# ZhonghuaYi/FocusFlow_official

Measured on AMD Instinct MI355X. Metric: frame-pairs/sec FF-RAFT 384x512 iters=12, higher is better.
Workload: dtype f32 via fp16x3 split operands on the f16 MFMA pipe (f32 accumulate, fp32-level accuracy); 1 GPU; FF-RAFT forward (test_mode), 8 pairs/GPU 384x512, iters=12, fp32 correlation pyramid, random-init weights, ORB-like masks (BASELINE configs[1]); pairs_per_gpu=8, corr_pyramid=fp32, conv_precision=f16x3, hipgraph=False, skip_unused_upsample=False, parallelism=dp1 (independent shards, no collective)

## Files before the change

focusflow_official_amd/_hip.py:

```python
import ctypes as C
import os

_PKG = os.path.dirname(os.path.abspath(__file__))
LIB_PATH = os.path.join(_PKG, "lib", "libfocusflow_hip.so")
if os.environ.get("FF_LAB_LIB"):
    LIB_PATH = os.path.join(_PKG, "lib", os.environ["FF_LAB_LIB"])

ACT_NONE, ACT_RELU, ACT_SIGMOID, ACT_TANH, ACT_LEAKY = 0, 1, 2, 3, 4
W_F32, W_F16X3, W_F16 = 0, 1, 2
MAX_SEG = 3
_fp = C.c_void_p
_ll = C.c_longlong


class FFFusionPair(C.Structure):
    _fields_ = [
        ("x", _fp * 2), ("x_ld", C.c_int * 2), ("xres", _fp * 2), ("xres_ld", C.c_int * 2), ("scale", _fp * 2), ("shift", _fp * 2),
        ("in_act", C.c_int), ("w_frag", _fp * 2), ("bias", _fp * 2), ("w_format", C.c_int), ("y", _fp * 2), ("y_ld", C.c_int * 2),
        ("B", C.c_int), ("HW", C.c_int), ("C", C.c_int),
    ]


class FFEncoderTail(C.Structure):
    _fields_ = [
# ... 83 lines not shown
    "ff_corr_alt_lookup": [_fp, C.POINTER(_fp), C.c_int, _fp, C.c_int, C.c_int, C.c_int, _fp, C.c_int, _fp, _fp],
    "ff_corr_alt_lookup_bwd": [_fp, C.POINTER(_fp), C.POINTER(_fp), C.POINTER(_fp), C.c_int, C.c_int, C.c_int, C.c_int, C.c_int, _fp,
                               C.POINTER(_fp), _fp],
    "ff_act_copy": [_fp, C.c_int, _fp, C.c_int, _ll, C.c_int, C.c_int, _fp],
    "ff_range_probe": [_fp, C.c_int, _ll, C.c_int, _fp, _fp],
    "ff_split_copy": [_fp, C.c_int, _fp, C.c_int, _ll, C.c_int, C.c_int, C.c_int, _fp],
    "ff_coords_init": [_fp, _fp, C.c_int, C.c_int, C.c_int, _fp],
    "ff_forward_interpolate": [_fp, _fp, _fp, C.c_int, C.c_int, C.c_int, _fp],
    "ff_good_features": [_fp, C.c_int, _ll, _ll, _ll, C.c_int, C.c_int, C.c_int, C.c_int, C.c_double, C.c_int, _fp, _fp, _fp, _fp, _fp],
    "ff_frame_ingest": [_fp, _ll, _ll, _ll, _ll, C.c_int, C.c_int, C.c_int, C.c_int, C.c_int, C.c_int, C.c_int, C.c_int, _fp, _fp],
    "ff_pad_replicate": [_fp, C.c_int, _ll, _ll, _ll, C.c_int, C.c_int, C.c_int, C.c_int, C.c_int, C.c_int, C.c_int, _fp, _fp],
    "ff_keypoint_matches": [_fp, _fp, C.c_int, _fp, _ll, _ll, _ll, _ll, C.c_int, C.c_int, C.c_int, C.c_int, C.c_int, C.c_int, C.c_int, _fp, _fp, _fp],
    "ff_tracks_replenish": [_fp, _fp, _fp, _fp, C.c_int, _fp, _fp, C.c_int, C.c_int, C.c_int, C.c_int, C.c_int, _fp, _fp, _fp],
    "ff_tracks_mask": [_fp, _fp, C.c_int, C.c_int, C.c_int, C.c_int, _fp, _fp],
    "ff_tracks_advance": [_fp, _fp, _fp, C.c_int, _fp, _ll, _ll, _ll, _ll, C.c_int, C.c_int, C.c_int, C.c_int, C.c_int, C.c_int, C.c_int, _fp, _fp, _fp,
                          _fp, _fp],
    "ff_fb_dense": [_fp, _ll, _ll, _ll, _ll, _fp, _ll, _ll, _ll, _ll, C.c_int, C.c_int, C.c_int, C.c_int, C.c_int, C.c_int, C.c_int, C.c_float, C.c_float,
                    _fp, _fp, _fp],
    "ff_fb_matches": [_fp, _fp, C.c_int, _fp, _ll, _ll, _ll, _ll, C.c_int, C.c_int, C.c_int, C.c_int, C.c_int, C.c_int, C.c_int, C.c_float, C.c_float,
                      _fp, _fp, _fp, _fp, _fp, _fp],
    "ff_epipolar_ransac": [_fp, _fp, C.c_int, C.c_int, C.c_int, C.c_int, C.c_float, C.c_int, C.c_int, C.c_int, C.c_uint, _fp, C.c_int, _fp, _fp, _fp, _fp,
                           _fp, _fp, _fp, _fp, _fp, _fp, _ll, _fp],
    "ff_epipolar_ransac_hold": [_fp, _fp, C.c_int, C.c_int, C.c_int, C.c_int, C.c_float, C.c_int, C.c_int, C.c_int, C.c_uint, _fp, C.c_int, _fp, _fp, _fp,
                                _fp, _fp, _fp, _fp, _fp, _fp, _fp, _ll, _fp, _fp],
    "ff_homography_ransac": [_fp, _fp, C.c_int, C.c_int, C.c_int, C.c_int, C.c_float, C.c_int, C.c_int, C.c_int, C.c_int, C.c_uint, _fp, C.c_int, _fp, _fp,
                             _fp, _fp, _fp, _fp, _fp, _fp, _fp, _fp, _fp, _ll, _fp],
    "ff_homography_residual": [_fp, _ll, _ll, _ll, _ll, _fp, _fp, C.c_int, C.c_int, C.c_int, _fp, _fp],
    "ff_coords_step": [_fp, _fp, C.c_int, _fp, _fp, C.c_int, C.c_int, C.c_int, C.c_int, _fp],
    "ff_gru_pass": [C.c_int, _fp, C.c_int, _fp, C.c_int, _fp, C.c_int, _fp, C.c_int, _fp, C.c_int, _fp, _fp, _fp, _fp, C.c_int, _fp, C.c_int, _fp, C.c_int,
                    C.c_int, C.c_int, C.c_int, _fp],
    "ff_gru_pass_rec": [C.c_int, _fp, C.c_int, _fp, C.c_int, _fp, C.c_int, _fp, C.c_int, _fp, C.c_int, _fp, _fp, _fp, _fp, C.c_int, _fp, C.c_int, _fp, C.c_int,
                        _fp, _fp, _fp, C.c_int, C.c_int, C.c_int, C.c_int, _fp],
    "ff_fusion_pair_fwd": [C.POINTER(FFFusionPair), _fp],
    "ff_encoder_tail_fwd": [C.POINTER(FFEncoderTail), _fp],
    "ff_conv_s2_pair_fwd": [C.POINTER(FFConvS2Pair), _fp],
    "ff_gru_rh": [_fp, C.c_int, _fp, C.c_int, _fp, C.c_int, _ll, C.c_int, _fp],
    "ff_gru_blend": [_fp, C.c_int, _fp, C.c_int, _fp, C.c_int, _fp, C.c_int, _ll, C.c_int, _fp],
    "ff_upsample_flow": [_fp, C.c_int, _fp, C.c_int, _fp, C.c_int, C.c_int, C.c_int, _fp],
    "ff_nhwc_to_nchw": [_fp, C.c_int, _fp, C.c_int, C.c_int, C.c_int, C.c_int, _fp],
    "ff_conv2d_wgrad": [C.POINTER(FFConvParams), _fp, _ll, _fp, _fp],
    "ff_unpack_conv_wgrad": [_fp, C.c_int, C.c_int, C.c_int, C.c_int, C.c_int, C.c_int, _fp, _fp],
    "ff_pack_conv_weight_dgrad": [_fp, C.c_int, C.c_int, C.c_int, C.c_int, _fp, C.c_int, C.c_int, _fp],
    "ff_act_bwd": [_fp, C.c_int, _fp, C.c_int, _fp, C.c_int, _ll, C.c_int, C.c_int, C.c_int, C.c_float, _fp, _fp],
    "ff_deconv4x4s2_small": [_fp, C.c_int, C.c_int, C.c_int, C.c_int, C.c_int, _fp, _fp, C.c_int, _fp, C.c_int, _fp],
    "ff_dilate2": [_fp, C.c_int, _fp, C.c_int, C.c_int, C.c_int, C.c_int, C.c_int, C.c_int, _fp],
    "ff_norm_bwd": [_fp, C.c_int, _fp, C.c_int, _fp, C.c_int, _fp, _fp, C.c_int, C.c_int, C.c_float, _fp, _fp,
                    C.c_int, _fp, C.c_int, _fp, C.c_int, C.c_int, C.c_int, C.c_int, _fp, _fp],
    "ff_gru_rh_bwd": [_fp, C.c_int, _fp, C.c_int, _fp, C.c_int, _fp, C.c_int, _fp, C.c_int, _ll, C.c_int, _fp],
    "ff_gru_blend_bwd": [_fp, C.c_int, _fp, C.c_int, _fp, C.c_int, _fp, C.c_int, _fp, C.c_int, _fp, C.c_int,
                         _fp, C.c_int, _ll, C.c_int, _fp],
    "ff_upsample_flow_bwd": [_fp, _fp, C.c_int, _fp, C.c_int, _fp, _fp, C.c_int, C.c_int, C.c_int, _fp],
    "ff_upsample_flow_bwd_ex": [_fp, _fp, C.c_int, _fp, C.c_int, _fp, C.c_int, _fp, C.c_float, _fp, C.c_int, C.c_int, C.c_int, _fp],
    "ff_gru_bwd_blend": [_fp, C.c_int, _fp, C.c_int, _fp, C.c_int, _fp, C.c_int, _fp, C.c_int, _fp, C.c_int, _fp, C.c_int, _fp, C.c_int, _fp, C.c_int,
                         _fp, _fp, _ll, C.c_int, _fp],
    "ff_gru_bwd_rh": [_fp, C.c_int, _fp, C.c_int, _fp, C.c_int, _fp, C.c_int, _fp, C.c_int, _fp, C.c_int, C.c_int, _fp, _ll, C.c_int, _fp],
    "ff_gru_bwd_out": [_fp, C.c_int, _fp, C.c_int, _fp, C.c_int, _fp, C.c_int, _fp, C.c_int, _fp, C.c_int, C.c_int, _fp, _ll, C.c_int, _fp],
    "ff_sum_stack": [_fp, C.c_int, _ll, _fp, _fp],
    "ff_pwc_costvolume_fwd": [_fp, C.c_int, _fp, C.c_int, _fp, C.c_int, C.c_int, C.c_int, C.c_int, C.c_int, _fp],
    "ff_pwc_costvolume_fwd_ex": [_fp, C.c_int, _fp, C.c_int, _fp, C.c_int, C.c_int, C.c_int, C.c_int, C.c_int, C.c_int, _fp, C.c_int, _fp],
    "ff_pwc_costvolume_bwd": [_fp, C.c_int, _fp, C.c_int, _fp, C.c_int, C.c_int, C.c_int, C.c_int, C.c_int, _fp],
    "ff_pwc_gout_transpose": [_fp, C.c_int, _fp, C.c_int, C.c_int, C.c_int, C.c_int, _fp],
    "ff_pwc_backwarp": [_fp, C.c_int, _fp, C.c_int, C.c_float, _fp, C.c_int, C.c_int, C.c_int, C.c_int, C.c_int, _fp],
    "ff_loss_prepare": [_fp, _fp, _fp, _fp, C.c_int, C.c_float, _fp, _fp, _fp, C.c_int, C.c_int, C.c_int, _fp],
    "ff_loss_accumulate": [_fp, _fp, _fp, _fp, _fp, C.c_float, C.c_float, C.c_float, _fp, _fp, C.c_int, C.c_int,
                           C.c_int, _fp],
    "ff_epe_metric": [_fp, _fp, _fp, _fp, C.c_int, C.c_int, C.c_int, _fp],
# ... 97 lines not shown
```

focusflow_official_amd/cce.py:

```python
from typing import Tuple, Optional, Sequence

import ctypes
import os
import weakref

import torch
import torch.nn as nn

from . import _hip, fn, ops
from .ops import ACT_NONE, ACT_RELU, ACT_SIGMOID

EPS = 1e-5


_NORM_ON_LOAD = True


_ALL_PACKED = weakref.WeakSet()
_DMA_FRAG = True
_PREPACK = True
_serial = [0]


class PackedConv:
# ... 276 lines not shown
            arr[i] = J
        host = torch.frombuffer(bytearray(bytes(arr)), dtype=torch.uint8)
        cache = owner.__dict__["_ff_pack_table"] = (sig, host.to(device), len(jobs), blk)
    ops.pack_weights_table(cache[1], cache[2], cache[3])
    for (pc, nf, nd, kf, kd), (J, fmt, dfmt) in zip(todo, jobs):
        if nf:
            pc.w, pc.fmt, pc._key = (pc._w_raw if fmt == 0 else pc._w_split), fmt, kf
            pc._gen += 1
        if nd:
            pc.wd, pc.dfmt, pc._dkey = (pc._wd_raw if dfmt == 0 else pc._wd_split), dfmt, kd
    return len(todo)


def train_streams() -> bool:
    v = os.environ.get("FF_TRAIN_STREAMS")
    if v is not None:
        return v != "0"
    return not (torch.distributed.is_available() and torch.distributed.is_initialized())
_BRANCH_STREAMS = True
_branch_streams = {}


def _branch_stream(device):
    key = (torch.device(device).index, torch.cuda.current_stream(device).cuda_stream)
    if key not in _branch_streams:
        _branch_streams[key] = torch.cuda.Stream(device=device)
    return _branch_streams[key]


_FUSION_PAIR = os.environ.get("FF_FUSION_PAIR", "1") != "0"
_PAIR_FUSION = True
_ENCODER_TAIL = True
_S2_PAIR = True
_W_LIMIT = 4094.0


def invalidate_packed(module: nn.Module) -> int:
    ids = {id(p) for p in module.parameters()}
    n = 0
    for pc in list(_ALL_PACKED):
        if id(pc.convs[0]._parameters["weight"]) in ids:
            pc._key = pc._dkey = None
            n += 1
    for m in module.modules():
        if hasattr(m, "_ff_fold"):
            del m._ff_fold
            n += 1
        if getattr(m, "_pair_key", None) is not None:
            m._pair_key = None
            n += 1
        if getattr(m, "_tail_key", None) is not None:
            m._tail_key = None
            n += 1
        if getattr(m, "_mask2_stage_of", None) is not None:
            m._mask2_stage = m._mask2_stage_of = None
            n += 1
    return n


def _make_norm(kind: str, c: int):
    if kind == "batch":
        return nn.BatchNorm2d(c)
    if kind == "instance":
        return nn.InstanceNorm2d(c)
    if kind == "none":
        return nn.Sequential()
# ... 76 lines not shown
            self.mask2img = _FusionConv(2 * c, c)
            self.img2mask = _FusionConv(2 * c, c) if bi_direction else None
        elif fusion_type in ("SA", "CA"):
            unit = _SA if fusion_type == "SA" else _CA
            self.mask2img = unit(c)
            self.img2mask = unit(c) if bi_direction else None
        else:
            raise ValueError(f"Fusion type {fusion_type} not supported.")

    def _paired(self):
        a, b = self.mask2img.conv, self.img2mask.conv
        key = (ops.conv_precision(),) + tuple((t._version, t.data_ptr()) for t in (a.weight, a.bias, b.weight, b.bias))
        if getattr(self, "_pair_key", None) != key:
            c = a.out_channels
            wf = torch.zeros((2 * c, 2 * c, 1, 1), dtype=torch.float32, device=a.weight.device)
            wf[:c, c:] = a.weight.detach()
            wf[c:, :c] = b.weight.detach()
            rows = torch.empty((2 * c, 2 * c), dtype=torch.float32, device=wf.device)
            ops.pack_conv_weight(wf, rows, 2 * c, 0)
            self._pair_w = ops.pack_split(rows)
            self._pair_b = torch.cat([a.bias.detach(), b.bias.detach()]).contiguous()
            self._pair_key = key
        return self._pair_w, self._pair_b

    def _pair_kernel_ok(self, img):
        if not (_FUSION_PAIR and self.fusion_type == "1x1conv" and self.img2mask is not None and not torch.is_grad_enabled()
                and ops.w_format() in (_hip.W_F16X3, _hip.W_F16)):
            return False
        b, h, w, c = img.shape
        tp = ops.fusion_pair_tile(c)
        return tp > 0 and (h * w) % tp == 0

    def run(self, mask, img):
        if self._pair_kernel_ok(img) and mask.shape == img.shape and ops.fusion_pair_inputs_ok(img, mask):
            pa, pb = self.mask2img._p, self.img2mask._p
            (_, ba), (_, bb) = pa.get(), pb.get()
            img_out, mask_out = ops.fusion_pair(img, mask, (pa.frag(), pb.frag()), (ba, bb), ops.w_format())
            return mask_out, img_out
        if isinstance(img, ops.LazyAct):
            img = img.materialise()
        if isinstance(mask, ops.LazyAct):
            mask = mask.materialise()
        if (_PAIR_FUSION and self.fusion_type == "1x1conv" and self.img2mask is not None and not torch.is_grad_enabled()
                and ops.w_format() != 0 and img.shape[3] % 32 == 0 and img.shape == mask.shape):
            c = img.shape[3]
            w, bias = self._paired()
            y = ops.conv2d([img, mask], w, bias, 2 * c, 1, 1, res=img, res2=mask, res_split=c, w_fmt=ops.w_format())
            return y[..., c:], y[..., :c]
        if self.fusion_type in ("SA", "CA"):
            img_out = self.mask2img.run(img, mask)
            mask_out = self.img2mask.run(mask, img) if self.img2mask is not None else mask
        elif self.fusion_type == "concat":
            img_out = fn.conv(self.mask2img._p, [img, mask])
            mask_out = fn.conv(self.img2mask._p, [mask, img]) if self.img2mask is not None else mask
        else:
            img_out = fn.conv(self.mask2img._p, mask, res=img)
            mask_out = fn.conv(self.img2mask._p, img, res=mask) if self.img2mask is not None else mask
        return mask_out, img_out


class _ResidualEncoder(nn.Module):

    def _frame_layers(self, in_channel, output_dim):
        self.norm1 = _make_norm(self.norm_fn, 64)
        self.conv1 = nn.Conv2d(in_channel, 64, 7, stride=2, padding=3)
        self.layer1 = self._stage(64, 64, 1)
        self.layer2 = self._stage(64, 96, 2)
        self.layer3 = self._stage(96, 128, 2)
        self.conv2 = nn.Conv2d(128, output_dim, 1)

    def _init_weights(self):
# ... 188 lines not shown
            return False
        probe = torch.empty((1, h, w, c), device="meta")
        return unit._pair_kernel_ok(probe)

    def _tail_eligible(self) -> bool:
        return (_ENCODER_TAIL and not torch.is_grad_enabled() and ops.w_format() in (_hip.W_F16X3, _hip.W_F16)
                and self.fusion_type in ("1x1conv", "1x1conv-unidirection") and self.fusion5.img2mask is None
                and (self.conv2.in_channels, self.conv2.out_channels) == (128, 256) and self.conv2.weight.is_cuda)

    def _tail_weights(self):
        f4, f5 = self.fusion4, self.fusion5
        convs = [f4.mask2img.conv, self.conv2, self.mask_conv2, f5.mask2img.conv] + ([f4.img2mask.conv] if f4.img2mask is not None else [])
        key = (ops.conv_precision(),) + tuple((t._version, t.data_ptr()) for cv in convs for t in (cv._parameters["weight"], cv._parameters["bias"]))
        if getattr(self, "_tail_key", None) != key:
            if torch.cuda.is_current_stream_capturing():
                return None
            w64 = lambda cv: cv.weight.detach().double().flatten(1)
            b64 = lambda cv: cv.bias.detach().double()
            a4, wx, wm, a5 = (w64(cv) for cv in convs[:4])
            w_x, w_m, bm = wx, wx @ a4 + a5 @ wm, b64(self.mask_conv2)
            if f4.img2mask is not None:
                w_x = wx + a5 @ (wm @ w64(f4.img2mask.conv))
                bm = wm @ b64(f4.img2mask.conv) + bm
            bias = wx @ b64(f4.mask2img.conv) + b64(self.conv2) + a5 @ bm + b64(f5.mask2img.conv)
            wf = torch.cat([w_x, w_m], 1).float()
            self._tail = None
            if float(wf.abs().max()) < _W_LIMIT:
                rows = torch.empty_like(wf)
                ops.pack_conv_weight(wf[:, :, None, None].contiguous(), rows, wf.shape[1], 0)
                self._tail = (ops.pack_frag16(ops.pack_split(rows), wf.shape[0]), bias.float().contiguous())
            self._tail_key = key
        return self._tail

    def forward(self, x, mask):
        b, hh, ww = x.shape[0], x.shape[1], x.shape[2]
        lz1 = self._lazy_for(self.fusion1, 64, hh // 2, ww // 2)
        lz2 = self._lazy_for(self.fusion2, 64, hh // 2, ww // 2)
        lz3 = self._lazy_for(self.fusion3, 96, hh // 4, ww // 4)
        m, x = self._branches(lambda t: self._conv_norm(t, self._mstem, self.mask_norm1, ACT_RELU, lazy=lz1),
                              lambda t: self._run_stem(t, lz1), mask, x)
        m, x = self.fusion1.run(m, x)
        m, x = self._branches(lambda t: self._run_stage(self.mask_layer1, t, lz2), lambda t: self._run_stage(self.layer1, t, lz2), m, x)
        m, x = self.fusion2.run(m, x)
        m, x = self._branches(lambda t: self._run_stage(self.mask_layer2, t, lz3), lambda t: self._run_stage(self.layer2, t, lz3), m, x)
        m, x = self.fusion3.run(m, x)
        tail = self._tail_weights() if self._tail_eligible() else None
        lz4 = tail is not None and self.norm_fn == "instance"
        m, x = self._branches(lambda t: self._run_stage(self.mask_layer3, t, lz4), lambda t: self._run_stage(self.layer3, t, lz4), m, x)
        if tail is not None and ops.encoder_tail_inputs_ok(x, m):
            return ops.encoder_tail(x, m, tail[0], tail[1], ops.w_format())
        m, x = self.fusion4.run(m, x)
        m, x = fn.conv(self._mout, m), self._run_out(x)
        m, x = self.fusion5.run(m, x)
        return x

    def freeze_self(self, mode):
        if mode == "parallel":
            for mod in (self.conv1, self.norm1, self.layer1, self.layer2, self.layer3, self.conv2):
                for p in mod.parameters():
                    p.requires_grad = False

    def copy_to_branch(self):
        self.mask_conv1.load_state_dict(self.conv1.state_dict())
        self.mask_layer1.load_state_dict(self.layer1.state_dict())
        self.mask_layer2.load_state_dict(self.layer2.state_dict())
        self.mask_layer3.load_state_dict(self.layer3.state_dict())
        self.mask_conv2.load_state_dict(self.conv2.state_dict())
```

focusflow_official_amd/csrc/fusion_pair.hip:

```cpp
#include <algorithm>
#include <cstdlib>
#include "ff_common.h"

namespace {

typedef float f32x4 __attribute__((ext_vector_type(4)));
typedef _Float16 f16x8 __attribute__((ext_vector_type(8)));
typedef _Float16 f16x4 __attribute__((ext_vector_type(4)));

__device__ __forceinline__ int PI16(int i) { return (i >= 4 && i < 12) ? 2 * (i - 4) : (i < 4 ? 2 * i + 1 : 2 * (i - 12) + 9); }

struct FArgs {
    FFFusionPair p;
    long long tiles;
};

template <int C, int TP, int TERMS>
__global__ __launch_bounds__(256) __attribute__((amdgpu_waves_per_eu(2, 2))) void fusion_pair_kernel(const FArgs a) {
    constexpr int G = C / 4;
    constexpr int PSTEP = (256 / G) / 8 * 8;
    constexpr int NACT = PSTEP * G;
    constexpr int NI = TP / PSTEP;
    constexpr int NCH = C / 32;
    constexpr int NPG = TP / 16;
    constexpr int NTW = C / 32;
    constexpr int PLANE = TP * 128;
    constexpr int SROW = 2 * C * 4 + 16;
    constexpr int TBYTES = TP * C * 4;
    static_assert((PSTEP == 8 || PSTEP == 16) && NACT % 64 == 0 && TP % PSTEP == 0 && C % 32 == 0 && TP % 16 == 0, "tile shape");
    extern __shared__ __attribute__((aligned(16))) char smem[];
    const FFFusionPair& p = a.p;
    const int tid = threadIdx.x, lane = tid & 63, wave = tid >> 6;
    const int i16 = lane & 15, g16 = lane >> 4;
    const int grp = tid % G, pl = tid / G;
    const bool loader = NACT == 256 || tid < NACT;

    const int nb = wave * (C / 2);
    const int ob = nb / C;
    const int ib = 1 - ob;
    const int lb = nb - ob * C;
    constexpr bool WRES = NTW * NCH <= 4 || TP <= 32;
    f32x4 wr[NTW][NCH][TERMS == 3 ? 2 : 1];
    f32x4 bias[NTW];
    const __amdgpu_buffer_rsrc_t rw = __builtin_amdgcn_make_buffer_rsrc(const_cast<void*>(p.w_frag[ob]), 0, (C / 16) * NCH * 2048, 0x00020000);
    auto load_w = [&]() {
#pragma unroll
        for (int v = 0; v < NTW; ++v) {
            const int tile = lb / 16 + v;
#pragma unroll
            for (int kc = 0; kc < NCH; ++kc) {
                wr[v][kc][0] = __builtin_bit_cast(f32x4, __builtin_amdgcn_raw_buffer_load_b128(rw, lane * 16, (tile * NCH + kc) * 2048, 0));
                if (TERMS == 3) wr[v][kc][TERMS == 3 ? 1 : 0] = __builtin_bit_cast(f32x4, __builtin_amdgcn_raw_buffer_load_b128(rw, lane * 16, (tile * NCH + kc) * 2048 + 1024, 0));
            }
        }
    };
    if (WRES) load_w();
    {
        const float* bp = p.bias[ob];
#pragma unroll
        for (int v = 0; v < NTW; ++v) {
            bias[v] = (f32x4){0.f, 0.f, 0.f, 0.f};
            if (bp) bias[v] = *reinterpret_cast<const f32x4*>(bp + lb + v * 16 + g16 * 4);
        }
    }
    const float xinv = ff::SPLIT_INV;
    const int nbytes = (int)(a.tiles * TBYTES);
    __amdgpu_buffer_rsrc_t rx[2], rr[2], ry[2];
#pragma unroll
    for (int br = 0; br < 2; ++br) {
        rx[br] = __builtin_amdgcn_make_buffer_rsrc(const_cast<float*>(p.x[br]), 0, nbytes, 0x00020000);
        rr[br] = __builtin_amdgcn_make_buffer_rsrc(const_cast<float*>(p.xres[br] ? p.xres[br] : p.x[br]), 0, nbytes, 0x00020000);
        ry[br] = __builtin_amdgcn_make_buffer_rsrc(p.y[br], 0, nbytes, 0x00020000);
    }
    const int voff = tid * 16;
    const int cc = (grp * 4) & 31, kcw = (grp * 4) >> 5;
    const int sw0 = (pl >> 1) & 7;
    const int wofs0 = kcw * PLANE + pl * 128 + (((cc >> 3) ^ sw0) << 4) + (cc & 7) * 2;
    const int wofs1 = kcw * PLANE + pl * 128 + (((4 + (cc >> 3)) ^ sw0) << 4) + (cc & 7) * 2;
    const int sofs = pl * SROW + grp * 16;

    for (long long tile = blockIdx.x; tile < a.tiles; tile += gridDim.x) {
        const int tb = (int)(tile * TBYTES);
        const int bimg = (int)(tile * TP / p.HW);
        f32x4 val[2][NI], rsd[2][NI];
#pragma unroll
        for (int br = 0; br < 2; ++br)
#pragma unroll
            for (int j = 0; j < NI; ++j) {
                if (!loader) continue;
                val[br][j] = __builtin_bit_cast(f32x4, __builtin_amdgcn_raw_buffer_load_b128(rx[br], voff, tb + j * (NACT * 16), 0));
                if (p.xres[br]) rsd[br][j] = __builtin_bit_cast(f32x4, __builtin_amdgcn_raw_buffer_load_b128(rr[br], voff, tb + j * (NACT * 16), 0));
            }
#pragma unroll
        for (int br = 0; br < 2; ++br) {
            if (!p.scale[br] || !loader) continue;
            const f32x4 sc = *reinterpret_cast<const f32x4*>(p.scale[br] + (long long)bimg * C + grp * 4);
            const f32x4 sh = *reinterpret_cast<const f32x4*>(p.shift[br] + (long long)bimg * C + grp * 4);
#pragma unroll
            for (int j = 0; j < NI; ++j) {
#pragma unroll
                for (int r = 0; r < 4; ++r) {
                    float o = fmaf(val[br][j][r], sc[r], sh[r]);
                    o = ff::apply_act(o, p.in_act);
                    if (p.xres[br]) { o += rsd[br][j][r]; o = o < 0.f ? 0.f : o; }
                    val[br][j][r] = o;
                }
            }
        }
#pragma unroll
        for (int br = 0; br < 2; ++br)
#pragma unroll
            for (int j = 0; j < NI; ++j) {
                if (!loader) continue;
                ff::ff_f16x4 h0, h1;
                ff::split_pair4(val[br][j], h0, h1);
                const int jx = (PSTEP == 8 && (j & 1)) ? 64 : 0;
                *reinterpret_cast<ff::ff_f16x4*>(smem + br * NCH * PLANE + j * PSTEP * 128 + (wofs0 ^ jx)) = h0;
                if (TERMS == 3) *reinterpret_cast<ff::ff_f16x4*>(smem + br * NCH * PLANE + j * PSTEP * 128 + (wofs1 ^ jx)) = h1;
            }
        if (!WRES) load_w();
        __syncthreads();
        f32x4 acc[NTW][NPG];
#pragma unroll
        for (int v = 0; v < NTW; ++v)
#pragma unroll
            for (int g = 0; g < NPG; ++g) acc[v][g] = (f32x4){0.f, 0.f, 0.f, 0.f};
        {
            const int pxl = PI16(i16), swl = (pxl >> 1) & 7;
            const char* fa = smem + ib * NCH * PLANE + pxl * 128 + ((g16 ^ swl) << 4);
            const char* fb = smem + ib * NCH * PLANE + pxl * 128 + (((4 + g16) ^ swl) << 4);
// ... 35 lines not shown
            for (int j = 0; j < NI; ++j) {
                if (!loader) continue;
                const f32x4 cv = *reinterpret_cast<const f32x4*>(smem + sofs + j * PSTEP * SROW + br * C * 4);
                f32x4 o;
#pragma unroll
                for (int r = 0; r < 4; ++r) o[r] = cv[r] + val[br][j][r];
                __builtin_amdgcn_raw_buffer_store_b128(__builtin_bit_cast(__attribute__((__vector_size__(4 * sizeof(unsigned)))) unsigned, o), ry[br], voff + tb + j * (NACT * 16), 0, 0);
            }
        __syncthreads();
    }
}

template <int C, int TP>
int launch(const FArgs& a, hipStream_t s) {
    constexpr int NCH = C / 32;
    constexpr size_t lds = std::max<size_t>((size_t)2 * NCH * TP * 128, (size_t)TP * (2 * C * 4 + 16));
    static const int per_cu = ff::tune_env("FF_FUSION_BLOCKS_PER_CU") ? std::max(1, atoi(ff::tune_env("FF_FUSION_BLOCKS_PER_CU"))) : 2;
    const unsigned blocks = (unsigned)std::min<long long>(a.tiles, 256ll * per_cu);
    if (a.p.w_format == FF_W_F16X3) {
        FF_ALLOW_DYNAMIC_LDS((&fusion_pair_kernel<C, TP, 3>), (int)lds);
        fusion_pair_kernel<C, TP, 3><<<blocks, 256, lds, s>>>(a);
    } else {
        FF_ALLOW_DYNAMIC_LDS((&fusion_pair_kernel<C, TP, 1>), (int)lds);
        fusion_pair_kernel<C, TP, 1><<<blocks, 256, lds, s>>>(a);
    }
    return ff::check_launch("ff_fusion_pair_fwd");
}

}

extern "C" int ff_fusion_pair_tile(int C) { return C == 64 ? 128 : (C == 96 ? 32 : 0); }

extern "C" int ff_fusion_pair_fwd(const FFFusionPair* pp, void* stream) {
    FF_REQUIRE(pp, "ff_fusion_pair_fwd: null argument");
    const FFFusionPair& p = *pp;
    const int tp = ff_fusion_pair_tile(p.C);
    FF_REQUIRE(tp > 0, "ff_fusion_pair_fwd: C = %d (64 or 96 channels per branch; other fusion units take ff_conv2d_fwd)", p.C);
    FF_REQUIRE(p.B > 0 && p.HW > 0 && p.HW % tp == 0, "ff_fusion_pair_fwd: B %d, HW %d: pixels per image must be a multiple of %d", p.B, p.HW, tp);
    FF_REQUIRE((long long)p.B * p.HW * p.C * 4 < (1ll << 31), "ff_fusion_pair_fwd: a tensor of 2 GiB or more");
    FF_REQUIRE(p.w_format == FF_W_F16X3 || p.w_format == FF_W_F16, "ff_fusion_pair_fwd: w_format %d (a split weight format)", p.w_format);
    FF_REQUIRE(p.in_act >= FF_ACT_NONE && p.in_act <= FF_ACT_TANH, "ff_fusion_pair_fwd: bad in_act %d", p.in_act);
    for (int i = 0; i < 2; ++i) {
        FF_REQUIRE(p.x[i] && p.y[i] && p.w_frag[i], "ff_fusion_pair_fwd: null tensor (branch %d)", i);
        FF_REQUIRE(p.x_ld[i] == p.C && p.y_ld[i] == p.C && ff::aligned16(p.x[i]) && ff::aligned16(p.y[i]) && ff::aligned16(p.w_frag[i]) && (!p.bias[i] || ff::aligned16(p.bias[i])),
                   "ff_fusion_pair_fwd: contiguous NHWC tensors (leading dimension == C) / 16-byte alignment (branch %d)", i);
        FF_REQUIRE(!p.xres[i] || (p.scale[i] && p.xres_ld[i] == p.C && ff::aligned16(p.xres[i])),
                   "ff_fusion_pair_fwd: xres needs scale / shift, leading dimension == C, 16-byte alignment (branch %d)", i);
        FF_REQUIRE(!p.scale[i] || (p.shift[i] && ff::aligned16(p.scale[i]) && ff::aligned16(p.shift[i])), "ff_fusion_pair_fwd: scale without shift / alignment (branch %d)", i);
        FF_REQUIRE(p.y[i] != p.x[1 - i] && (!p.xres[1 - i] || p.y[i] != p.xres[1 - i]), "ff_fusion_pair_fwd: an output aliases the other branch's input");
    }
    FArgs a;
    a.p = p;
    a.tiles = (long long)p.B * p.HW / tp;
    hipStream_t s = static_cast<hipStream_t>(stream);
    return p.C == 64 ? launch<64, 128>(a, s) : launch<96, 32>(a, s);
}
```

focusflow_official_amd/model.py:

```python
import numpy as np
import torch
import torch.nn as nn

from . import _hip, ops
from .raft_net import RAFT

MASK_MODES = {"neighborG": 0, "neighborE": 1, "context": 2}


def gaussian_table(kernel_size, sigma):
    s3 = 3 * sigma
    xs = np.linspace(-s3, s3, kernel_size)
    x, y = np.meshgrid(xs, xs)
    gauss = 1 / (2 * np.pi * sigma ** 2) * np.exp(-(x ** 2 + y ** 2) / (2 * sigma ** 2))
    return torch.FloatTensor((1 / gauss.sum()) * gauss).contiguous()


def ellipse_table(k):
    r = c = k // 2
    el = np.zeros((k, k), np.float32)
    inv_r2 = 1.0 / (r * r) if r else 0.0
    for i in range(k):
        dy = i - r
        if abs(dy) <= r:
# ... 44 lines not shown
            self.flow_net.load_model(load_raft, flag="all", strict=False)
            print("Load all flow net.")
        if self.freeze_flownet:
            self.freeze_self()
            print("freeze flow net.")

    def invalidate_packed(self) -> int:
        from .cce import invalidate_packed
        self.flow_net._guard_hist, self.flow_net._guard_level, self.flow_net._exact_ctx = False, 0.0, False
        return invalidate_packed(self)

    def load_state_dict(self, *args, **kwargs):
        out = super().load_state_dict(*args, **kwargs)
        self.invalidate_packed()
        big = [k for k, v in self.state_dict().items() if v.dim() == 4 and float(v.abs().max()) >= 4094.0] if ops.w_format() else []
        if big:
            raise ValueError(f"conv weights beyond the range of the f16x3 split format (|w| >= 4094): {big[:3]}; "
                             "use FF_CONV_PRECISION=fp32 for this checkpoint")
        return out

    def train(self, mode: bool = True):
        self.invalidate_packed()
        return super().train(mode)

    def forward(self, image1, image2, mask1=None, mask2=None, raft_iters=12, flow_init=None, test_mode=False):
        b, c, h, w = image1.shape
        if h % 8 or w % 8:
            raise ValueError("H and W must be multiples of 8 (pad with InputPadder as the reference's callers do)")
        modal = self.mask_modal
        assert modal is None or mask1.shape[1] == 1
        i12 = ops.empty_nhwc(2 * b, h, w, 4, image1)
        i1 = ops.prep_input(image1, b, h, w, image1, out=i12[:b])
        i2 = ops.prep_input(image2, b, h, w, image1, out=i12[b:])
        if modal is None:
            m1 = m2 = None
        elif modal == "point":
            m12 = ops.empty_nhwc(2 * b, h, w, 4, image1)
            m1 = ops.prep_input(mask1, b, h, w, image1, out=m12[:b])
            m2 = ops.prep_input(None, b, h, w, image1, fill=255.0, out=m12[b:])
        elif modal == "frame":
            m1, m2 = i1, i2
        else:
            if self._table is None or self._table.device != image1.device:
                t = self.cfg.TRAIN
                tab = gaussian_table(t.KERNEL_SIZE, t.KERNEL_SIGMA) if modal == "neighborG" else ellipse_table(t.MASK_DILATE)
                self._table = tab.to(image1.device)
            m1 = ops.mask_prepare(MASK_MODES[modal], mask1, image1, self._table)
            m2 = i2 if modal == "context" else ops.prep_input(None, b, h, w, image1, fill=255.0)
        ops.guard_begin(image1.device)
        self.flow_net._guard_handled = False
        out = self.flow_net(i1, i2, m1, m2, iters=raft_iters, flow_init=flow_init, test_mode=test_mode)
        ops.guard_end("FF_RAFT_FUSION.forward", owner=self.flow_net, handled=self.flow_net._guard_handled)
        ops.check_range("FF_RAFT_FUSION.forward")
        return out

    def check_range(self):
        ops.guard_check(sync=True)

    def freeze_self(self):
        if self.use_fusion == "parallel":
            self.flow_net.freeze_self(mode="parallel")
```

focusflow_official_amd/ops.py:

```python
import ctypes as C
import math
import os
import threading
from typing import List, Optional, Sequence

import torch

from . import _hip
from ._hip import ACT_LEAKY, ACT_NONE, ACT_RELU, ACT_SIGMOID, ACT_TANH, FFConvParams

Tensor = torch.Tensor


_raw_stream = getattr(torch._C, "_cuda_getCurrentRawStream", None)
_raw_device = getattr(torch._C, "_cuda_getDevice", None)


def _stream():
    if _raw_stream is not None and _raw_device is not None:
        return C.c_void_p(_raw_stream(_raw_device()))
    return C.c_void_p(torch.cuda.current_stream().cuda_stream)


_PRECISIONS = {"fp32": _hip.W_F32, "f16x3": _hip.W_F16X3, "f16": _hip.W_F16}
# ... 1222 lines not shown

    @property
    def shape(self):
        return self.t.shape

    def coeffs(self):
        if self._coef is None:
            self._coef = norm_coeffs(self.stats, self.count, self.eps)
        return self._coef

    def materialise(self) -> Tensor:
        return norm_apply(self.t, self.stats, True, self.eps, act=self.act, res=self.res, out=self.t)

    def record_stream(self, stream):
        for x in (self.t, self.stats, self.res) + (tuple(self._coef) if self._coef is not None else ()):
            if x is not None:
                x.record_stream(stream)


def fusion_pair_tile(c: int) -> int:
    return _hip.load().ff_fusion_pair_tile(c)


def fusion_pair_inputs_ok(*ins) -> bool:
    for v in ins:
        for t in ((v.t, v.res) if isinstance(v, LazyAct) else (v,)):
            if t is not None and (not t.is_cuda or _ld(t) != t.shape[3] or t.numel() * 4 >= (1 << 31)):
                return False
    return True


def fusion_pair(img, mask, w_frag, bias, w_fmt: int):
    ins = (img, mask)
    b, h, w, c = ins[0].shape
    assert ins[1].shape == ins[0].shape
    p = _hip.FFFusionPair()
    outs = []
    for i, v in enumerate(ins):
        t = v.t if isinstance(v, LazyAct) else v
        _require_gpu(t)
        p.x[i], p.x_ld[i] = t.data_ptr(), _ld(t)
        if isinstance(v, LazyAct):
            sc, sh = v.coeffs()
            p.scale[i], p.shift[i] = sc.data_ptr(), sh.data_ptr()
            p.in_act = v.act
            if v.res is not None:
                p.xres[i], p.xres_ld[i] = v.res.data_ptr(), _ld(v.res)
        y = t if isinstance(v, LazyAct) else empty_nhwc(b, h, w, c, t)
        outs.append(y)
        p.y[i], p.y_ld[i] = y.data_ptr(), _ld(y)
        p.w_frag[i] = w_frag[i].data_ptr()
        p.bias[i] = bias[i].data_ptr() if bias[i] is not None else None
    if _range_word is not None:
        for v in ins:
            probe = v.res if isinstance(v, LazyAct) else v
            if probe is not None:
                _range_probe(probe)
    acts = {v.act for v in ins if isinstance(v, LazyAct)}
    assert len(acts) <= 1, "lazy inputs of one fusion unit share the activation"
    p.w_format, p.B, p.HW, p.C = w_fmt, b, h * w, c
    _timed_call("conv", "ff_fusion_pair_fwd", C.byref(p), _stream(), note=(2.0 * b * h * w * 2 * c * c, w_fmt))
    return outs[0], outs[1]


def encoder_tail_inputs_ok(*ins) -> bool:
    if not fusion_pair_inputs_ok(*ins) or ins[0].shape != ins[1].shape:
        return False
    b, h, w, c = ins[0].shape
    return c == 128 and b * h * w * 256 * 4 < (1 << 31) and all((v.t if isinstance(v, LazyAct) else v).dtype == torch.float32 for v in ins)


def encoder_tail(x, m, w_frag: Tensor, bias: Tensor, w_fmt: int) -> Tensor:
    ins = (x, m)
    b, h, w, c = ins[0].shape
    p = _hip.FFEncoderTail()
    for i, v in enumerate(ins):
        t = v.t if isinstance(v, LazyAct) else v
        _require_gpu(t)
        if tuple(t.shape[:3]) != (b, h, w):
            raise _hip.FocusFlowHipError(f"encoder_tail: inputs of different shapes {tuple(ins[0].shape)} / {tuple(t.shape)}")
        c = min(c, t.shape[3])
        p.x[i], p.x_ld[i] = t.data_ptr(), _ld(t)
        if isinstance(v, LazyAct):
            sc, sh = v.coeffs()
            p.scale[i], p.shift[i] = sc.data_ptr(), sh.data_ptr()
            p.in_act = v.act
            if v.res is not None:
                p.xres[i], p.xres_ld[i] = v.res.data_ptr(), _ld(v.res)
    acts = {v.act for v in ins if isinstance(v, LazyAct)}
    assert len(acts) <= 1, "lazy inputs of one stage share the activation"
    if _range_word is not None:
        for v in ins:
            probe = v.res if isinstance(v, LazyAct) else v
            if probe is not None:
# ... 350 lines not shown
```

focusflow_official_amd/raft_net.py:

```python
import os

import torch
import torch.nn as nn

from . import _hip, cce, corr_block, fn, ops, train_loop
from .cce import BasicEncoder, BasicParallelFusionLayer, train_streams
from .corr_block import AlternateCorrBlock, CorrBlock
from .ops import ACT_RELU, ACT_TANH
from .update_block import BasicUpdateBlock, split_activations

_COORDS_EPILOGUE = True
_MASK_UPSAMPLE = True
_GRU_CTX_ONCE = True
_STREAMS_MIN_PIXELS = int(os.environ.get("FF_STREAMS_MIN_PIXELS", "700000"))
_ENC_STREAMS = True


class RAFT(nn.Module):
    def __init__(self, in_channels=3, small=False, dropout=0., alternate_corr=False, abandon_fnet=False,
                 inside_fusion=None, fuse_cnet=False, cfg=None):
        super().__init__()
        if small or abandon_fnet or inside_fusion not in (None, "parallel"):
            raise NotImplementedError(
                f"RAFT(small={small}, abandon_fnet={abandon_fnet}, inside_fusion={inside_fusion!r}): the HIP path builds "
# ... 89 lines not shown
        ops.guard_probe(cnet, 0)
        ops.guard_probe(f12, 1)
        if ops.guard_careful(self):
            m_ctx, m_fmap = ops.guard_read_now()
            ops.guard_note(self, m_ctx, m_fmap)
            self._guard_handled = True
            if not (m_fmap < ops.X_LIMIT) or not (m_ctx < float("inf")):
                raise _hip.FocusFlowHipError(
                    f"RAFT.forward: an encoder output reached |x| = {max(m_ctx, m_fmap):.6g}; the fp16-split conv formats need |x| < {ops.X_LIMIT:g} "
                    "(csrc/ff_common.h).  Feature maps beyond it have no local exact route (the correlation values they produce overflow the "
                    "next layer as well), and an infinite context output means a layer INSIDE the encoder overflowed.  Run this checkpoint / "
                    "input with FF_CONV_PRECISION=fp32.")
            if not (m_ctx < ops.X_LIMIT) and not self._exact_ctx:
                if fn.recording(cnet):
                    raise _hip.FocusFlowHipError(
                        f"RAFT.forward: the context encoder's output reached |x| = {m_ctx:.6g} (limit {ops.X_LIMIT:g}) in a RECORDED pass; the "
                        "exact-fp32 repair covers inference only.  Train this checkpoint with FF_CONV_PRECISION=fp32.")
                import warnings
                warnings.warn(f"FF-RAFT: the context encoder's output reached |x| = {m_ctx:.6g} (limit of the fp16-split conv formats: "
                              f"{ops.X_LIMIT:g}); the convolutions that read it run on the exact-fp32 MFMA route from now on")
                self._exact_ctx = True
        taped = fn.recording(cnet)
        if taped:
            net = fn.ActFn.apply(cnet[..., :128], ACT_TANH)
            inp = fn.ActFn.apply(cnet[..., 128:], ACT_RELU)
        else:
            net = ops.empty_nhwc(b, h8, w8, 128, cnet)
            inp = ops.empty_nhwc(b, h8, w8, 128, cnet)
            ops.act_copy(cnet[..., :128], net, ACT_TANH)
            ops.act_copy(cnet[..., 128:], inp, ACT_RELU)
        coords1 = ops.coords_init(b, h8, w8, cnet, flow_init)
        return self._update_loop(net, inp, fmap1, fmap2, coords1, iters, loop_gate, corr_fn, test_mode)

    def _fused_train(self, test_mode=False) -> bool:
        return (torch.is_grad_enabled() and train_loop.ENABLED and _GRU_CTX_ONCE and ops.w_format() in (_hip.W_F16X3, _hip.W_F16)
                and not test_mode)

    def _loop_gate(self, fused_train):
        if fused_train and train_loop.defer_param_grads():
            lp = train_loop.loop_params(self.update_block)
            if all(q is None or q.is_cuda for q in lp) and any(q is not None and q.requires_grad for q in lp):
                box = {}
                return box, train_loop.LoopParamGate.apply(box, *lp)
        return None

    def _corr_block(self, fmap1, fmap2, fused_train):
        on_the_fly = self.alternate_corr
        if on_the_fly and fn.recording(fmap1, fmap2):
            if not self._alt_warned:
                import warnings
                warnings.warn("alternate_corr=True: the feature maps are recorded (trained encoders) - a recorded batch whose "
                              f"materialised all-pairs pyramid stays under {corr_block._MAX_PYRAMID_BYTES / 1e9:.2f} GB uses that "
                              "pyramid (the faster lookup); larger batches use the on-the-fly correlation and its backward")
                self._alt_warned = True
            b, h, w, _ = fmap1.shape
            on_the_fly = not corr_block.pyramid_fits(b, h, w, self.corr_pyramid_dtype)
        if fused_train:
            fmap1, fmap2 = fmap1.detach(), fmap2.detach()
        if on_the_fly:
            return AlternateCorrBlock(fmap1, fmap2, radius=self.corr_radius)
        return CorrBlock(fmap1, fmap2, radius=self.corr_radius, pyramid_dtype=self.corr_pyramid_dtype)

    def _update_loop(self, net, inp, fmap1, fmap2, coords1, iters, loop_gate=None, corr_fn=None, test_mode=False):
        b, h8, w8, _ = net.shape
        fused_train = self._fused_train(test_mode)
        if corr_fn is None:
# ... 60 lines not shown
```

include/focusflow_hip.h:

```cpp
#ifndef FOCUSFLOW_HIP_H
#define FOCUSFLOW_HIP_H

#ifdef __cplusplus
extern "C" {
#endif

#define FF_OK 0
#define FF_EINVAL (-1)
#define FF_EHIP (-2)

#define FF_ACT_NONE 0
#define FF_ACT_RELU 1
#define FF_ACT_SIGMOID 2
#define FF_ACT_TANH 3
#define FF_ACT_LEAKY 4

#define FF_MAX_SEG 3

#define FF_W_F32 0
#define FF_W_F16X3 1
#define FF_W_F16 2

const char* ff_last_error(void);
#define FF_ABI_VERSION 7
// ... 163 lines not shown
                            int min_inliers, int permille, unsigned int seed, int* epoch, int cull, float* pos, long long* ids,
                            int* age, float* F, float* dist2, unsigned char* status, int* inliers, int* candidates,
                            unsigned char* ok, void* ws, long long ws_size, const unsigned char* hold, void* stream);
int ff_homography_ws(int B, int N, int K);
int ff_homography_ransac(const float* matches, unsigned char* valid, int B, int N, int H, int W, float threshold, int K, int min_inliers,
                         int permille, int planar_permille, unsigned int seed, int* epoch, int cull, float* pos, long long* ids,
                         int* age, float* Hm, float* dist2, unsigned char* status, int* inliers, int* candidates, unsigned char* ok,
                         unsigned char* planar, void* ws, long long ws_size, void* stream);
int ff_homography_residual(const float* flow, long long ld_b, long long ld_c, long long ld_row, long long ld_col, const float* Hm,
                           const unsigned char* ok, int B, int Himg, int Wimg, float* out, void* stream);
int ff_coords_step(float* coords1, const float* delta, int delta_ld, float* flow4,
                   float* slot, int slot_ld, int B, int H, int W, void* stream);
int ff_gru_pass(int dir, const float* hs, int hs_ld, const float* motion, int mo_ld, const float* h, int h_ld,
                const float* zr_pre, int zr_pre_ld, const float* q_pre, int q_pre_ld, const void* wzr_frag, const void* wq_frag,
                const float* bzr, const float* bq, int w_format, float* y, int y_ld, float* y2, int y2_ld, int B, int H, int W,
                void* stream);
int ff_gru_pass_rec(int dir, const float* hs, int hs_ld, const float* motion, int mo_ld, const float* h, int h_ld,
                    const float* zr_pre, int zr_pre_ld, const float* q_pre, int q_pre_ld, const void* wzr_frag, const void* wq_frag,
                    const float* bzr, const float* bq, int w_format, float* y, int y_ld, float* y2, int y2_ld, float* z, float* r,
                    float* q, int gate_ld, int B, int H, int W, void* stream);
typedef struct FFFusionPair {
    const float* x[2];     int x_ld[2];
    const float* xres[2];  int xres_ld[2];
    const float* scale[2]; const float* shift[2];
    int in_act;
    const void* w_frag[2];
    const float* bias[2];
    int w_format;
    float* y[2];           int y_ld[2];
    int B, HW, C;
} FFFusionPair;
int ff_fusion_pair_tile(int C);
int ff_fusion_pair_fwd(const FFFusionPair* p, void* stream);
typedef struct FFEncoderTail {
    const float* x[2];     int x_ld[2];
    const float* xres[2];  int xres_ld[2];
    const float* scale[2]; const float* shift[2];
    int in_act;
    const void* w_frag;
    const float* bias;
    int w_format;
    float* y;              int y_ld;
    int B, HW, C, Cout;
} FFEncoderTail;
int ff_encoder_tail_fwd(const FFEncoderTail* p, void* stream);
typedef struct FFConvS2Pair {
    const float* x;        int x_ld;
    int B, H, W, Cin, Cout;
    int k[2], stride[2], pad[2];
    const void* w3_frag;   const void* w1_frag;
    int w_format;
    const float* bias[2];  const float* scale[2]; const float* shift[2];
    int act[2];
    float* y[2];           int y_ld[2];
    float* stats_part[2];
} FFConvS2Pair;
int ff_conv_s2_pair_stats_parts(int H, int W);
int ff_conv_s2_pair_fwd(const FFConvS2Pair* p, void* stream);
int ff_gru_rh(const float* r, int r_ld, const float* h, int h_ld, float* rh, int rh_ld,
              long long npix, int C, void* stream);
int ff_gru_blend(const float* z, int z_ld, const float* q, int q_ld, const float* h, int h_ld,
                 float* h_new, int hn_ld, long long npix, int C, void* stream);
int ff_mask_upsample_pack(const void* w_split, void* w_stage, void* stream);
int ff_mask_upsample_fwd(const float* hid, int hid_ld, const void* w_stage, int w_format, const float* bias, float out_scale,
                         const float* flow, int flow_ld, float* out, int B, int H, int W, void* stream);
int ff_upsample_flow(const float* flow, int flow_ld, const float* mask, int mask_ld,
// ... 124 lines not shown
```

Baseline: 638.9 frame-pairs/s.

## Share a single constant second-frame mask image across the batch in the fusion encoder

For the point and neighbor modalities, the second frame's condition mask is a constant 255 fill, so it is now prepared once instead of once per pair. The mask branch of the parallel fusion encoder then runs on b+1 images instead of 2b. A new ff_fusion_pair_fwd_n entry point clamps each branch's image index so the fused 1x1 fusion-pair kernel can read a shorter mask batch and still produce full-batch outputs. This removes redundant mask-encoder convolutions and input preparation, at the cost of extra guard logic, alias checks, and a hard error for fusion units that cannot take a shorter mask batch.

```diff
diff --git a/focusflow_official_amd/_hip.py b/focusflow_official_amd/_hip.py
--- a/focusflow_official_amd/_hip.py
+++ b/focusflow_official_amd/_hip.py
@@ -139,6 +139,7 @@
     "ff_gru_pass_rec": [C.c_int, _fp, C.c_int, _fp, C.c_int, _fp, C.c_int, _fp, C.c_int, _fp, C.c_int, _fp, _fp, _fp, _fp, C.c_int, _fp, C.c_int, _fp, C.c_int,
                         _fp, _fp, _fp, C.c_int, C.c_int, C.c_int, C.c_int, _fp],
     "ff_fusion_pair_fwd": [C.POINTER(FFFusionPair), _fp],
+    "ff_fusion_pair_fwd_n": [C.POINTER(FFFusionPair), C.POINTER(C.c_int), _fp],
     "ff_encoder_tail_fwd": [C.POINTER(FFEncoderTail), _fp],
     "ff_conv_s2_pair_fwd": [C.POINTER(FFConvS2Pair), _fp],
     "ff_gru_rh": [_fp, C.c_int, _fp, C.c_int, _fp, C.c_int, _ll, C.c_int, _fp],
diff --git a/focusflow_official_amd/cce.py b/focusflow_official_amd/cce.py
--- a/focusflow_official_amd/cce.py
+++ b/focusflow_official_amd/cce.py
@@ -332,6 +332,7 @@
 _PAIR_FUSION = True
 _ENCODER_TAIL = True
 _S2_PAIR = True
+_SHARED_MASK2 = True
 _W_LIMIT = 4094.0
 
 
@@ -474,11 +475,15 @@
         return tp > 0 and (h * w) % tp == 0
 
     def run(self, mask, img):
-        if self._pair_kernel_ok(img) and mask.shape == img.shape and ops.fusion_pair_inputs_ok(img, mask):
+        short = mask.shape[0] < img.shape[0]
+        if self._pair_kernel_ok(img) and tuple(mask.shape[1:]) == tuple(img.shape[1:]) and mask.shape[0] <= img.shape[0] and ops.fusion_pair_inputs_ok(img, mask):
             pa, pb = self.mask2img._p, self.img2mask._p
             (_, ba), (_, bb) = pa.get(), pb.get()
             img_out, mask_out = ops.fusion_pair(img, mask, (pa.frag(), pb.frag()), (ba, bb), ops.w_format())
             return mask_out, img_out
+        if short:
+            raise _hip.FocusFlowHipError(f"FusionUnit: {mask.shape[0]} condition images for {img.shape[0]} frames, and ff_fusion_pair_fwd_n "
+                                         "does not take this unit")
         if isinstance(img, ops.LazyAct):
             img = img.materialise()
         if isinstance(mask, ops.LazyAct):
@@ -733,8 +738,15 @@
             self._tail_key = key
         return self._tail
 
+    def shared_mask2_ok(self, frames, hh, ww) -> bool:
+        return (_SHARED_MASK2 and frames > 2 and hh % 2 == 0 and ww % 2 == 0 and self._lazy_for(self.fusion1, 64, hh // 2, ww // 2)
+                and frames * (hh // 2) * (ww // 2) * 64 * 4 < (1 << 31))
+
     def forward(self, x, mask):
         b, hh, ww = x.shape[0], x.shape[1], x.shape[2]
+        self.cond_images = mask.shape[0]
+        if mask.shape[0] != b and not (mask.shape[0] < b and self.shared_mask2_ok(b, hh, ww)):
+            raise _hip.FocusFlowHipError(f"BasicParallelFusionLayer: {mask.shape[0]} condition images for {b} frames (shared_mask2_ok says when fewer are read)")
         lz1 = self._lazy_for(self.fusion1, 64, hh // 2, ww // 2)
         lz2 = self._lazy_for(self.fusion2, 64, hh // 2, ww // 2)
         lz3 = self._lazy_for(self.fusion3, 96, hh // 4, ww // 4)
diff --git a/focusflow_official_amd/csrc/fusion_pair.hip b/focusflow_official_amd/csrc/fusion_pair.hip
--- a/focusflow_official_amd/csrc/fusion_pair.hip
+++ b/focusflow_official_amd/csrc/fusion_pair.hip
@@ -13,6 +13,7 @@
 struct FArgs {
     FFFusionPair p;
     long long tiles;
+    int n_img[2];
 };
 
 template <int C, int TP, int TERMS>
@@ -65,11 +66,13 @@
     }
     const float xinv = ff::SPLIT_INV;
     const int nbytes = (int)(a.tiles * TBYTES);
+    const int ibytes = p.HW * C * 4;
     __amdgpu_buffer_rsrc_t rx[2], rr[2], ry[2];
 #pragma unroll
     for (int br = 0; br < 2; ++br) {
-        rx[br] = __builtin_amdgcn_make_buffer_rsrc(const_cast<float*>(p.x[br]), 0, nbytes, 0x00020000);
-        rr[br] = __builtin_amdgcn_make_buffer_rsrc(const_cast<float*>(p.xres[br] ? p.xres[br] : p.x[br]), 0, nbytes, 0x00020000);
+        const int xbytes = a.n_img[br] * ibytes;
+        rx[br] = __builtin_amdgcn_make_buffer_rsrc(const_cast<float*>(p.x[br]), 0, xbytes, 0x00020000);
+        rr[br] = __builtin_amdgcn_make_buffer_rsrc(const_cast<float*>(p.xres[br] ? p.xres[br] : p.x[br]), 0, xbytes, 0x00020000);
         ry[br] = __builtin_amdgcn_make_buffer_rsrc(p.y[br], 0, nbytes, 0x00020000);
     }
     const int voff = tid * 16;
@@ -82,20 +85,26 @@
     for (long long tile = blockIdx.x; tile < a.tiles; tile += gridDim.x) {
         const int tb = (int)(tile * TBYTES);
         const int bimg = (int)(tile * TP / p.HW);
+        int bi[2], tbx[2];
+#pragma unroll
+        for (int br = 0; br < 2; ++br) {
+            bi[br] = min(bimg, a.n_img[br] - 1);
+            tbx[br] = tb - (bimg - bi[br]) * ibytes;
+        }
         f32x4 val[2][NI], rsd[2][NI];
 #pragma unroll
         for (int br = 0; br < 2; ++br)
 #pragma unroll
             for (int j = 0; j < NI; ++j) {
                 if (!loader) continue;
-                val[br][j] = __builtin_bit_cast(f32x4, __builtin_amdgcn_raw_buffer_load_b128(rx[br], voff, tb + j * (NACT * 16), 0));
-                if (p.xres[br]) rsd[br][j] = __builtin_bit_cast(f32x4, __builtin_amdgcn_raw_buffer_load_b128(rr[br], voff, tb + j * (NACT * 16), 0));
+                val[br][j] = __builtin_bit_cast(f32x4, __builtin_amdgcn_raw_buffer_load_b128(rx[br], voff, tbx[br] + j * (NACT * 16), 0));
+                if (p.xres[br]) rsd[br][j] = __builtin_bit_cast(f32x4, __builtin_amdgcn_raw_buffer_load_b128(rr[br], voff, tbx[br] + j * (NACT * 16), 0));
             }
 #pragma unroll
         for (int br = 0; br < 2; ++br) {
             if (!p.scale[br] || !loader) continue;
-            const f32x4 sc = *reinterpret_cast<const f32x4*>(p.scale[br] + (long long)bimg * C + grp * 4);
-            const f32x4 sh = *reinterpret_cast<const f32x4*>(p.shift[br] + (long long)bimg * C + grp * 4);
+            const f32x4 sc = *reinterpret_cast<const f32x4*>(p.scale[br] + (long long)bi[br] * C + grp * 4);
+            const f32x4 sh = *reinterpret_cast<const f32x4*>(p.shift[br] + (long long)bi[br] * C + grp * 4);
 #pragma unroll
             for (int j = 0; j < NI; ++j) {
 #pragma unroll
@@ -197,7 +206,12 @@
 extern "C" int ff_fusion_pair_tile(int C) { return C == 64 ? 128 : (C == 96 ? 32 : 0); }
 
 extern "C" int ff_fusion_pair_fwd(const FFFusionPair* pp, void* stream) {
-    FF_REQUIRE(pp, "ff_fusion_pair_fwd: null argument");
+    const int all[2] = {0, 0};
+    return ff_fusion_pair_fwd_n(pp, all, stream);
+}
+
+extern "C" int ff_fusion_pair_fwd_n(const FFFusionPair* pp, const int* n_img, void* stream) {
+    FF_REQUIRE(pp && n_img, "ff_fusion_pair_fwd: null argument");
     const FFFusionPair& p = *pp;
     const int tp = ff_fusion_pair_tile(p.C);
     FF_REQUIRE(tp > 0, "ff_fusion_pair_fwd: C = %d (64 or 96 channels per branch; other fusion units take ff_conv2d_fwd)", p.C);
@@ -215,6 +229,20 @@
         FF_REQUIRE(p.y[i] != p.x[1 - i] && (!p.xres[1 - i] || p.y[i] != p.xres[1 - i]), "ff_fusion_pair_fwd: an output aliases the other branch's input");
     }
     FArgs a;
+    const long long ibytes = (long long)p.HW * p.C * 4;
+    for (int i = 0; i < 2; ++i) {
+        a.n_img[i] = n_img[i] ? n_img[i] : p.B;
+        FF_REQUIRE(a.n_img[i] >= 1 && a.n_img[i] <= p.B, "ff_fusion_pair_fwd: n_img[%d] = %d (0, or 1 .. B = %d)", i, n_img[i], p.B);
+        FF_REQUIRE(a.n_img[i] * ibytes < (1ll << 31), "ff_fusion_pair_fwd: a tensor of 2 GiB or more (branch %d)", i);
+        if (a.n_img[i] < p.B) {
+            const char *y0 = reinterpret_cast<const char*>(p.y[i]), *y1 = y0 + p.B * ibytes;
+            for (const float* in : {p.x[i], p.xres[i]}) {
+                const char* x0 = reinterpret_cast<const char*>(in);
+                FF_REQUIRE(!in || x0 + a.n_img[i] * ibytes <= y0 || y1 <= x0,
+                           "ff_fusion_pair_fwd: the output of a branch with n_img < B aliases that branch's input (branch %d: %d of %d images)", i, a.n_img[i], p.B);
+            }
+        }
+    }
     a.p = p;
     a.tiles = (long long)p.B * p.HW / tp;
     hipStream_t s = static_cast<hipStream_t>(stream);
diff --git a/focusflow_official_amd/model.py b/focusflow_official_amd/model.py
--- a/focusflow_official_amd/model.py
+++ b/focusflow_official_amd/model.py
@@ -100,12 +100,13 @@
         i12 = ops.empty_nhwc(2 * b, h, w, 4, image1)
         i1 = ops.prep_input(image1, b, h, w, image1, out=i12[:b])
         i2 = ops.prep_input(image2, b, h, w, image1, out=i12[b:])
+        b2 = 1 if modal in ("point", "neighborG", "neighborE") and self.flow_net.shared_mask2_ok(b, h, w) else b
         if modal is None:
             m1 = m2 = None
         elif modal == "point":
-            m12 = ops.empty_nhwc(2 * b, h, w, 4, image1)
+            m12 = ops.empty_nhwc(b + b2, h, w, 4, image1)
             m1 = ops.prep_input(mask1, b, h, w, image1, out=m12[:b])
-            m2 = ops.prep_input(None, b, h, w, image1, fill=255.0, out=m12[b:])
+            m2 = ops.prep_input(None, b2, h, w, image1, fill=255.0, out=m12[b:])
         elif modal == "frame":
             m1, m2 = i1, i2
         else:
@@ -114,7 +115,7 @@
                 tab = gaussian_table(t.KERNEL_SIZE, t.KERNEL_SIGMA) if modal == "neighborG" else ellipse_table(t.MASK_DILATE)
                 self._table = tab.to(image1.device)
             m1 = ops.mask_prepare(MASK_MODES[modal], mask1, image1, self._table)
-            m2 = i2 if modal == "context" else ops.prep_input(None, b, h, w, image1, fill=255.0)
+            m2 = i2 if modal == "context" else ops.prep_input(None, b2, h, w, image1, fill=255.0)
         ops.guard_begin(image1.device)
         self.flow_net._guard_handled = False
         out = self.flow_net(i1, i2, m1, m2, iters=raft_iters, flow_init=flow_init, test_mode=test_mode)
diff --git a/focusflow_official_amd/ops.py b/focusflow_official_amd/ops.py
--- a/focusflow_official_amd/ops.py
+++ b/focusflow_official_amd/ops.py
@@ -1278,8 +1278,9 @@
 
 def fusion_pair(img, mask, w_frag, bias, w_fmt: int):
     ins = (img, mask)
-    b, h, w, c = ins[0].shape
-    assert ins[1].shape == ins[0].shape
+    n_img = (ins[0].shape[0], ins[1].shape[0])
+    b, (_, h, w, c) = max(n_img), ins[0].shape
+    assert tuple(ins[1].shape[1:]) == tuple(ins[0].shape[1:])
     p = _hip.FFFusionPair()
     outs = []
     for i, v in enumerate(ins):
@@ -1292,7 +1293,7 @@
             p.in_act = v.act
             if v.res is not None:
                 p.xres[i], p.xres_ld[i] = v.res.data_ptr(), _ld(v.res)
-        y = t if isinstance(v, LazyAct) else empty_nhwc(b, h, w, c, t)
+        y = t if isinstance(v, LazyAct) and n_img[i] == b else empty_nhwc(b, h, w, c, t)
         outs.append(y)
         p.y[i], p.y_ld[i] = y.data_ptr(), _ld(y)
         p.w_frag[i] = w_frag[i].data_ptr()
@@ -1305,7 +1306,10 @@
     acts = {v.act for v in ins if isinstance(v, LazyAct)}
     assert len(acts) <= 1, "lazy inputs of one fusion unit share the activation"
     p.w_format, p.B, p.HW, p.C = w_fmt, b, h * w, c
-    _timed_call("conv", "ff_fusion_pair_fwd", C.byref(p), _stream(), note=(2.0 * b * h * w * 2 * c * c, w_fmt))
+    if n_img[0] == n_img[1]:
+        _timed_call("conv", "ff_fusion_pair_fwd", C.byref(p), _stream(), note=(2.0 * b * h * w * 2 * c * c, w_fmt))
+    else:
+        _timed_call("conv", "ff_fusion_pair_fwd_n", C.byref(p), (C.c_int * 2)(*n_img), _stream(), note=(2.0 * b * h * w * 2 * c * c, w_fmt))
     return outs[0], outs[1]
 
 
diff --git a/focusflow_official_amd/raft_net.py b/focusflow_official_amd/raft_net.py
--- a/focusflow_official_amd/raft_net.py
+++ b/focusflow_official_amd/raft_net.py
@@ -145,6 +145,9 @@
         coords1 = ops.coords_init(b, h8, w8, cnet, flow_init)
         return self._update_loop(net, inp, fmap1, fmap2, coords1, iters, loop_gate, corr_fn, test_mode)
 
+    def shared_mask2_ok(self, b, hh, ww) -> bool:
+        return isinstance(self.fnet, BasicParallelFusionLayer) and self.fnet.shared_mask2_ok(2 * b, hh, ww)
+
     def _fused_train(self, test_mode=False) -> bool:
         return (torch.is_grad_enabled() and train_loop.ENABLED and _GRU_CTX_ONCE and ops.w_format() in (_hip.W_F16X3, _hip.W_F16)
                 and not test_mode)
diff --git a/include/focusflow_hip.h b/include/focusflow_hip.h
--- a/include/focusflow_hip.h
+++ b/include/focusflow_hip.h
@@ -219,6 +219,7 @@
 } FFFusionPair;
 int ff_fusion_pair_tile(int C);
 int ff_fusion_pair_fwd(const FFFusionPair* p, void* stream);
+int ff_fusion_pair_fwd_n(const FFFusionPair* p, const int n_img[2], void* stream);
 typedef struct FFEncoderTail {
     const float* x[2];     int x_ld[2];
     const float* xres[2];  int xres_ld[2];
```

Result: no change. 641.5 frame-pairs/s, median of 6 (+0.4%).
